# savage-hacker14/audio-to-sheet-music

Hardware: AMD Instinct MI355X
Metric: 6s-segments/sec (each separated into 4 stems; encode once, decode 4x) (higher is better)
Workload: dtype bf16; 1 GPU; BASELINE configs[2]: B=64 x 6 s segments x 4 prompts per GPU; global_batch=64, seq_len=264600, prompts=4, parallelism=segment-sharded dp1, launch=hipGraph replay of one athd_forward_prompts per step (1 graph(s) per rank), pipelines=1, decode_items=256

## Files before the change

### audio-to-sheet-music_amd/csrc/forward.h

```cpp
#pragma once
#include <hip/hip_runtime.h>

#include <algorithm>
#include <cstdio>
#include <cstdlib>
#include <string>
#include <vector>

#include "../../include/athd.h"
#include "attn.h"
#include "ctx.h"
#include "gemm.h"
#include "kernels.h"
#include "prof.h"

namespace athd_fwd {

struct Dims {
    int64_t B = 0, T = 0;
    int P = 1, Tspec = 0;
    int F[5] = {2048, 512, 128, 32, 8};
    int64_t L[5] = {0, 0, 0, 0, 0};
    int64_t Nf = 0, Nt = 0, Nmax = 0;
    int64_t Bc = 0, chunks = 0;
// ... 19 lines not shown
    float *avec, *tc0, *tc2;
    float *Yb, *x_cond, *xt_cond;
    void* Hm;
    float* Ybt;
    void* Hmt;
    float *G, *D, *FO;
    float* FO2 = nullptr;
    float* ola_part;
    LrStep* lrsteps;
    float* gram;
    double* gramq;
    void *S, *Z, *Zs;
    float* skw[2] = {nullptr, nullptr};
};

inline void* eoff(void* p, int64_t n, int ea) { return (char*)p + n * ea; }

struct Switches {
    static bool env(const char* name, bool dflt) {
        const char* e = std::getenv(name);
        return dflt ? !(e && *e == '0') : (e && *e && *e != '0');
    }
    bool serial = env("ATHD_SERIAL", false), sk = env("ATHD_SK", true), rowln = env("ATHD_ROWLN", true),
         fdec1_fused = env("ATHD_FDEC1_FUSED", true), fenc_row = env("ATHD_FENC_ROW", true);
};

struct Status {
    int err = 0;
    std::string what;
    void check(int rc, const char* w) { if (rc != 0 && err == 0) { err = rc; what = w; } }
};

enum Branch { MAIN = 0, TIME = 1 };
struct StreamPlan {
    hipStream_t main, time;
    hipEvent_t ev_f, ev_t;
    bool serial;
    Status* st;

    StreamPlan(athd_ctx* c, hipStream_t caller, bool serial_, Status* st_)
        : main(caller), time(serial_ ? caller : c->s_time), ev_f(c->ev_f), ev_t(c->ev_t), serial(serial_), st(st_) {
        if (!c->s_time || !c->ev_f || !c->ev_t) st->check((int)hipErrorInvalidResourceHandle, "second stream");
    }
    void record(hipEvent_t ev, hipStream_t s) { st->check((int)hipEventRecord(ev, s), "event record"); }
    void wait(hipStream_t s, hipEvent_t ev) { st->check((int)hipStreamWaitEvent(s, ev, 0), "event wait"); }
    void fork() { record(ev_f, main); wait(time, ev_f); }
    void join() { record(ev_t, time); wait(main, ev_t); }
// ... 74 lines not shown
```

### audio-to-sheet-music_amd/csrc/forward_xf.cpp

```cpp
#include "forward.h"

namespace athd_fwd {
namespace {

struct Pending { const double* st = nullptr; const float* w = nullptr; const float* b = nullptr; };

struct BranchX {
    float* X;
    int64_t N;
    void *QKV, *O, *F1;
    Pending pend;
    Pending resgn;
};

struct Xf {
    Run& r;
    const Dims& d;
    const Bufs& b;
    const int ab;

    void ln(BranchX& x, const float* w, const float* bb, bool pending, void* out, const float* w2 = nullptr,
            const float* b2 = nullptr, void* out2 = nullptr) {
        LnDesc l;
        l.x = x.X; l.nb = (int)d.B; l.N = x.N; l.C = 512; l.w = w; l.b = bb; l.out = out; l.out_bf16 = ab;
// ... 49 lines not shown
        GemmDesc g2 = lin(L.l2, x.F1, ab, B, N, 2048, x.X, 0);
        g2.res = x.X; g2.res_scale = L.g2; g2.stats = st;
        g2.sk_ws = r.sw.sk ? b.skw[r.sk] : nullptr;
        r.gemm(g2, "linear2");
        x.pend.st = st; x.pend.w = L.now; x.pend.b = L.nob;
    }
    void down(const GemmW& w, BranchX& x, float* enc, uint16_t* enc_b, const char* site) {
        GemmDesc g = lin(w, x.X, 0, d.B, x.N, 512, enc, 0);
        if (r.actbf) { g.a_gn_stats = x.pend.st; g.a_gn_count = x.N * 512; g.a_gn_w = x.pend.w; g.a_gn_b = x.pend.b; }
        r.gemm(g, site);
        if (enc_b) to_bf16_launch(enc, enc_b, d.B * x.N * 384, r.s);
    }
};

}

void transformer(Run& r, const Dims& d, const Bufs& b) {
    athd_ctx* c = r.c;
    KStage xstage("transformer");
    KSection sec_x("transformer");
    const int64_t B = d.B;
    Xf xf{r, d, b, r.actbf ? 1 : 0};
    BranchX f{b.X, d.Nf, b.QKV, b.O, b.F1}, t{b.XT, d.Nt, b.QKVt, b.Ot, b.F1t};
    r.gemm(lin(c->up, b.saved[3], xf.ab, B, d.Nf, 384, b.X, 0), "upsampler");
    r.gemm(lin(c->up_t, b.saved_t[3], xf.ab, B, d.Nt, 384, b.XT, 0), "upsampler_t");
    pos2d_launch(b.pos2d, 8, d.Tspec, 512, r.s);
    pos1d_launch(b.pos1d, (int)d.Nt, 512, r.s);
    LnDesc l;
    l.x = b.X; l.nb = (int)B; l.N = d.Nf; l.C = 512; l.w = c->nin_w; l.b = c->nin_b; l.pos = b.pos2d; l.out = b.X;
    layernorm_launch(l, r.s);
    LnDesc lt;
    lt.x = b.XT; lt.nb = (int)B; lt.N = d.Nt; lt.C = 512; lt.w = c->nint_w; lt.b = c->nint_b; lt.pos = b.pos1d; lt.out = b.XT;
    layernorm_launch(lt, r.s);
    if (!r.ok()) return;
    r.sp.fork();
    for (int idx = 0; idx < 5; ++idx) {
        const TLayerW& Lf = c->L[idx];
        const TLayerW& Lt = c->Lt[idx];
        if (!Lf.cross) {
            xf.ln(f, Lf.n1w, Lf.n1b, true, b.H[0]);
            xf.block(Lf, f, b.H[0], nullptr, d.Nf);
            OnBranch on(r, TIME);
            xf.ln(t, Lt.n1w, Lt.n1b, true, b.H[2]);
            xf.block(Lt, t, b.H[2], nullptr, d.Nt);
        } else {
            r.sp.cross_join();
            xf.ln(f, Lf.n1w, Lf.n1b, true, b.H[0], Lt.n2w, Lt.n2b, b.H[1]);
            {
                OnBranch on(r, TIME);
                xf.ln(t, Lt.n1w, Lt.n1b, true, b.H[2], Lf.n2w, Lf.n2b, b.H[3]);
            }
            r.sp.cross_join();
            xf.block(Lf, f, b.H[0], b.H[3], d.Nt);
            OnBranch on(r, TIME);
            xf.block(Lt, t, b.H[2], b.H[1], d.Nf);
        }
    }
    if (!r.actbf) gn_apply_launch(b.X, (int)B, d.Nf, 512, f.pend.st, f.pend.w, f.pend.b, r.s);
    {
        OnBranch on(r, TIME);
        if (!r.actbf) gn_apply_launch(b.XT, (int)B, d.Nt, 512, t.pend.st, t.pend.w, t.pend.b, r.s);
        xf.down(c->down_t, t, b.xt_enc, b.xt_enc_b, "downsampler_t");
    }
    xf.down(c->down, f, b.x_enc, b.x_enc_b, "downsampler");
    r.sp.join();
}
// ... 3 lines not shown
```

### audio-to-sheet-music_amd/csrc/gemm.h

```cpp
#pragma once
#include <hip/hip_runtime.h>
#include <stdint.h>

namespace athd {

enum Act { ACT_NONE = 0, ACT_GELU = 1, ACT_GLU = 2 };

struct FastDivU {
    uint32_t mul = 0, shift = 0, d = 1;
};
inline FastDivU make_fastdiv(uint32_t d) {
    FastDivU f;
    f.d = d;
    if (d <= 1) return f;
    uint32_t l = 0;
    while ((1ull << l) < d) ++l;
    f.mul = (uint32_t)((((uint64_t)1 << (31 + l)) + d - 1) / d);
    f.shift = l - 1;
    return f;
}
#if defined(__HIPCC__)
__device__ inline uint32_t fdiv(uint32_t n, const FastDivU& f) { return f.d == 1 ? n : __umulhi(n, f.mul) >> f.shift; }
#endif

// ... 32 lines not shown
    int act = ACT_NONE;
    const void* res = nullptr;
    int res_bf16 = 0;
    const float* res_scale = nullptr;
    const double* res_gn_stats = nullptr;
    int64_t res_gn_count = 0;
    const float* res_gn_w = nullptr;
    const float* res_gn_b = nullptr;
    const float* row_add = nullptr;
    double* stats = nullptr;
    const double* gn_stats = nullptr;
    FastDivU fd_w, fd_h, fd_hw;
    int64_t gn_count = 0;
    const float* gn_w = nullptr;
    const float* gn_b = nullptr;
    const float* pbias = nullptr;
    int pfold = 1, res_div = 1;
    int64_t res_bs = 0;
    const float* ln_w = nullptr;
    const float* ln_b = nullptr;
    void* ln_out = nullptr;
    float* sk_ws = nullptr;
    int sk_full = 0, sk_S = 1;
};

constexpr int SK_MAX_PIECES = 320;
constexpr size_t SK_WS_BYTES = (size_t)SK_MAX_PIECES * 256 * 256 * 4;

inline void gemm_work(const GemmDesc& d, int mode, double& flops, double& bytes) {
    const double M = (double)d.nb * d.H_out * d.W;
    flops = 2.0 * M * d.N * d.K;
    const double nout = d.act == ACT_GLU ? d.N / 2 : d.N;
    bytes = (double)d.nb * d.H_in * d.W * d.C_in * (d.a_bf16 ? 2 : 4) + (double)d.N * d.K * (mode == 1 ? 2 : 4);
    if (d.store) bytes += M * nout * (d.c_bf16 ? 2 : 4) * (d.pfold > 1 ? d.pfold : 1);
    if (d.res) bytes += M * nout * (d.res_bf16 ? 2 : 4) / (d.res_div > 1 ? d.res_div : 1);
    if (d.pbias) bytes += (double)d.nb * (d.pfold > 1 ? d.pfold : 1) * d.N * 4;
}

enum GemmRoute {
    ROUTE_REFUSED = 0,
    ROUTE_ROWLN,
    ROUTE_ROWLN_TEXT,
    ROUTE_GEMM3_LN,
    ROUTE_GEMM2_AGN,
    ROUTE_GEMM5,
    ROUTE_GEMM3_V3,
    ROUTE_GEMM3_V7,
    ROUTE_GEMM2,
    ROUTE_V1_BF16,
    ROUTE_V1_F32
};

int gemm_launch(const GemmDesc& d, int mode, hipStream_t s);
int gemm_route(const GemmDesc& d, int mode);
struct SkPlan {
    int full, tail, S;
};
SkPlan gemm5_sk_plan(const GemmDesc& d, int64_t R);
int64_t gemm5_sk_resident(const GemmDesc& d);
bool rowln_supported(const GemmDesc& d);
inline GemmDesc with_fastdiv(const GemmDesc& d) {
    GemmDesc e = d;
    e.fd_w = make_fastdiv((uint32_t)d.W);
    e.fd_h = make_fastdiv((uint32_t)d.H_out);
    e.fd_hw = make_fastdiv((uint32_t)d.H_out * (uint32_t)d.W);
    return e;
}

}
```

### audio-to-sheet-music_amd/csrc/gemm.hip

```cpp
#include <cstdlib>

#include "gemm_launch.h"

namespace athd {

constexpr int BK = 32;

template <int MODE> struct CT;
template <> struct CT<0> { typedef float T; };
template <> struct CT<1> { typedef bf16_t T; };

typedef __attribute__((ext_vector_type(8))) __bf16 bf16v8;

template <typename T> struct Vec8 { T v[8]; };

template <int MODE, int BM, int BN, int WM, int WN, bool VEC8>
__global__ __launch_bounds__(256) void gemm_kernel(const GemmDesc d) {
    using T = typename CT<MODE>::T;
    constexpr int PAD = (MODE == 1) ? 8 : 4;
    constexpr int LD = BK + PAD;
    constexpr int TM = BM / WM / 16;
    constexpr int TN = BN / WN / 16;
    constexpr int AROWS = BM / 64;
    constexpr int BGROUPS = (BN * 4 + 255) / 256;
// ... 215 lines not shown
}

template <int MODE, int BM, int BN, int WM, int WN>
static void launch_cfg(const GemmDesc& d, hipStream_t s) {
    const int64_t M = (int64_t)d.nb * d.H_out * d.W;
    dim3 grid((unsigned)((M + BM - 1) / BM), (unsigned)((d.N + BN - 1) / BN));
    const bool vec8 = (d.C_in % 8 == 0) && (d.a_ld % 8 == 0) && d.a_cs == 1;
    GemmScope ks(s, d, MODE, "gemm_kernel<%d,%d,%d,%d,%d,%s>", MODE, BM, BN, WM, WN, vec8 ? "true" : "false");
    if (vec8) hipLaunchKernelGGL((gemm_kernel<MODE, BM, BN, WM, WN, true>), grid, dim3(256), 0, s, with_fastdiv(d));
    else hipLaunchKernelGGL((gemm_kernel<MODE, BM, BN, WM, WN, false>), grid, dim3(256), 0, s, with_fastdiv(d));
}

template <int MODE>
static void launch_mode(const GemmDesc& d, hipStream_t s) {
    if (d.N <= 16 && d.act != ACT_GLU) launch_cfg<MODE, 256, 16, 4, 1>(d, s);
    else if (d.N <= 32) launch_cfg<MODE, 256, 32, 4, 1>(d, s);
    else if (d.N <= 64) launch_cfg<MODE, 128, 64, 2, 2>(d, s);
    else launch_cfg<MODE, 128, 128, 2, 2>(d, s);
}

int gemm_route(const GemmDesc& d, int mode) {
    if (d.Kp % BK != 0 || d.Kp < d.K || d.C_in <= 0 || d.N <= 0) return ROUTE_REFUSED;
    if (d.act == ACT_GLU && (d.N % 32 != 0)) return ROUTE_REFUSED;
    if (d.ln_out) return mode == 1 && rowln_supported(d) ? ROUTE_ROWLN : ROUTE_REFUSED;
    if (d.ln_w) {
        if (mode != 1) return ROUTE_REFUSED;
        if (rowln_text_enabled() && rowln_text_supported(d)) return ROUTE_ROWLN_TEXT;
        return gemm3_ln_supported(d) ? ROUTE_GEMM3_LN : ROUTE_REFUSED;
    }
    if (d.a_gn_stats) return mode == 1 && gemm2_supported(d) ? ROUTE_GEMM2_AGN : ROUTE_REFUSED;
    if (d.res_gn_stats && !(mode == 1 && gemm5_supported(d) && d.N % 256 == 0 && epi_res_fast_ok(d))) return ROUTE_REFUSED;
    if (mode == 1 && gemm5_supported(d) && d.N % 256 == 0) return ROUTE_GEMM5;
    if (mode == 1 && gemm3_supported(d) && d.N >= 192) return d.K >= 384 ? ROUTE_GEMM3_V7 : ROUTE_GEMM3_V3;
    if (mode == 1 && gemm2_supported(d)) return ROUTE_GEMM2;
    return mode == 1 ? ROUTE_V1_BF16 : ROUTE_V1_F32;
}

int gemm_launch(const GemmDesc& d0, int mode, hipStream_t s) {
    const GemmDesc d = with_fastdiv(d0);
#ifdef ATHD_KBENCH
    if (mode == 1 && gemm_route(d, mode) >= ROUTE_GEMM5) {
        const int rc = gemm6_launch(d, s);
        if (rc != -2) return rc;
    }
#endif
    const GemmRoute route = (GemmRoute)gemm_route(d, mode);
    switch (route) {
        case ROUTE_ROWLN: return rowln_launch(d, s);
        case ROUTE_ROWLN_TEXT: return rowln_text_launch(d, s);
        case ROUTE_GEMM3_LN: return gemm3_ln_launch(d, s);
        case ROUTE_GEMM2_AGN:
        case ROUTE_GEMM2: return gemm2_launch(d, s);
        case ROUTE_GEMM5: return gemm5_launch(d, s);
        case ROUTE_GEMM3_V3:
        case ROUTE_GEMM3_V7: return gemm3_launch(d, s, route);
        case ROUTE_V1_BF16: launch_mode<1>(d, s); return (int)hipGetLastError();
        case ROUTE_V1_F32: launch_mode<0>(d, s); return (int)hipGetLastError();
        default: return -2;
    }
}

}
```

### audio-to-sheet-music_amd/csrc/gemm_launch.h

```cpp
#pragma once
#include "common.h"
#include "prof.h"
#include "gemm.h"
#include "gemm_epi.h"

#include <type_traits>

namespace athd {

bool gemm2_supported(const GemmDesc& d);
int gemm2_launch(const GemmDesc& d, hipStream_t s);
bool gemm3_supported(const GemmDesc& d);
int gemm3_launch(const GemmDesc& d, hipStream_t s, GemmRoute route);
bool gemm3_ln_supported(const GemmDesc& d);
int gemm3_ln_launch(const GemmDesc& d, hipStream_t s);
bool gemm5_supported(const GemmDesc& d);
int gemm5_launch(const GemmDesc& d, hipStream_t s);
int rowln_launch(const GemmDesc& d, hipStream_t s);
bool rowln_text_enabled();
bool rowln_text_supported(const GemmDesc& d);
int rowln_text_launch(const GemmDesc& d, hipStream_t s);
#ifdef ATHD_KBENCH
int gemm3_variant_launch(const GemmDesc& d, hipStream_t s, int variant);
int gemm4_launch(const GemmDesc& d, hipStream_t s);
int gemm5_probe_launch(const GemmDesc& d, hipStream_t s, int probe);
int gemm6_launch(const GemmDesc& d, hipStream_t s);
#endif

template <auto Kernel>
int64_t resident_blocks(int threads) {
    static int per_cu = 0;
    if (per_cu == 0) {
        (void)hipOccupancyMaxActiveBlocksPerMultiprocessor(&per_cu, Kernel, threads, 0);
        if (per_cu <= 0) per_cu = -1;
    }
    return per_cu > 0 ? (int64_t)per_cu * device_cus() : 0;
}

template <typename Fn>
void dispatch_epi(unsigned flags, Fn&& f) {
    switch (flags) {
// ... 20 lines not shown
```

### audio-to-sheet-music_amd/csrc/ktest.cpp

```cpp
#include <hip/hip_runtime.h>
#include <stdint.h>
#include <string.h>

#include "attn.h"
#include "ctx.h"
#include "gemm.h"
#include "kernels.h"

namespace athd {
bool dconv_conv3_supported(int C, int H, int kp, int64_t L);
bool dconv_apply_supported(int C, int H, int kp, int64_t M);
int dec_merge_run();
int dec_merge_maxp();
int dec_last_const(int which);
int fdec1_gram_wb();
int fdec1_gram_blocks();
}

using namespace athd;

extern "C" {

struct KtGemm {
    void* A; int64_t a_bf16, nb, H_in, W, C_in, a_ld, a_cs, a_bs, a_hs, ntaps, in_stride, in_off, dil, H_out;
    void* a_norm; void* a_gn_stats; int64_t a_gn_count; void* a_gn_w; void* a_gn_b;
    void* Wp; int64_t N, K, Kp; void* bias;
    void* C; int64_t c_bf16, H_out_total, o_stride, o_off, ldo, col_off, c_bs, store; void* c4;
    int64_t col_split, hi_row_off, store_mask, k_blk, act;
    void* res; int64_t res_bf16; void* res_scale; void* res_gn_stats; int64_t res_gn_count; void* res_gn_w; void* res_gn_b;
    void* row_add; void* stats; void* gn_stats; int64_t gn_count; void* gn_w; void* gn_b;
    void* pbias; int64_t pfold, res_div, res_bs;
    void* ln_w; void* ln_b; void* ln_out; void* sk_ws;
};

struct KtAttn {
    void* Q; int64_t q_bf16, q_bs, q_ld, q_off;
    void* K; int64_t k_bf16, k_bs, k_ld, k_off;
    void* V; int64_t v_bf16, v_bs, v_ld, v_off;
    void* O; int64_t o_bf16, o_bs, o_ld;
// ... 258 lines not shown
    d.H_skip2 = (int)k->H_skip2; d.C_skip2 = (int)k->C_skip2;
    return d;
}
int kt_fdec_last(const KtDecLast* k, void* stream) { return fdec_last_launch(to_dl(k), (hipStream_t)stream); }
int kt_tdec_last(const KtDecLast* k, void* stream) { return tdec_last_launch(to_dl(k), (hipStream_t)stream); }
int kt_fdec_tail(const KtDecLast* k, void* stream) { return fdec_tail_launch(to_dl(k), (hipStream_t)stream); }
int kt_tdec_tail(const KtDecLast* k, void* stream) { return tdec_tail_launch(to_dl(k), (hipStream_t)stream); }
int kt_tdec_tail_supported(const KtDecLast* k) { return tdec_tail_supported(to_dl(k)); }
int64_t kt_fl_dc() { return dec_last_const(0); }
int64_t kt_ft_dc() { return dec_last_const(1); }
int64_t kt_tl_in() { return dec_last_const(2); }
int64_t kt_tt_rows() { return dec_last_const(3); }
int64_t kt_dm_run() { return dec_merge_run(); }
int64_t kt_merge_maxp() { return dec_merge_maxp(); }
int64_t kt_g_wb() { return fdec1_gram_wb(); }
int64_t kt_fdec1_gram_blocks() { return fdec1_gram_blocks(); }
int64_t kt_dec_last_fold(const float* w, const float* b, const float* P, const float* pb, int64_t br, float* out) {
    const std::vector<float> f = dec_last_fold(std::vector<float>(w, w + 48 * 4 * 8), std::vector<float>(b, b + 4),
                                               std::vector<float>(P, P + 8), std::vector<float>(pb, pb + 2), (int)br);
    if (out) memcpy(out, f.data(), f.size() * sizeof(float));
    return (int64_t)f.size();
}

int kt_gn_apply(float* x, int64_t nb, int64_t N, int64_t C, const double* stats, const float* w, const float* b,
                void* stream) {
    gn_apply_launch(x, (int)nb, N, (int)C, stats, w, b, (hipStream_t)stream);
    return (int)hipGetLastError();
}

}
```

### audio-to-sheet-music_amd/csrc/rowln.hip

```cpp
#include "gemm_launch.h"
#include "gemm_tile.h"

namespace athd {

namespace {

constexpr int RL_N = 512, RL_K = 512;
constexpr int RT_N = 384, RT_K = 384;
constexpr int RL_NS = 3;
template <int KS, int TN, int AQ>
struct RlSched {
    static constexpr int KT = KS / 2;
    static constexpr int step(int ks) { return (ks + 1 < KS ? TN : 0) + ((ks % 2 == 0 && ks / 2 + 2 < KT) ? AQ : 0); }
    static constexpr int through(int ks) {
        int n = TN + 2 * AQ;
        for (int k = 0; k <= ks; ++k) n += step(k);
        return n;
    }
    static constexpr int pos_b(int k) {
        if (k == 0) return TN;
        return through(k - 2) + TN;
    }
    static constexpr int pos_a(int t) {
        if (t < 2) return TN + (t + 1) * AQ;
        return through(2 * (t - 2) - 1) + TN + AQ;
    }
    static constexpr int wait_b(int ks) { return through(ks) - pos_b(ks); }
    static constexpr int wait_a(int ks) { return through(ks) - pos_a(ks / 2 + 1); }
};

}

#ifndef ATHD_RL_RD
#define ATHD_RL_RD 2
#endif
#ifndef ATHD_RL_PROBE
#define ATHD_RL_PROBE 0
#endif

template <int BM, int NW, int N, int K, bool TEXT>
__global__ __launch_bounds__(64 * NW, 2) void rowln_kernel(const GemmDesc d) {
    constexpr int NT = 64 * NW;
    constexpr int RL_N = N, RL_K = K;
    constexpr int RL_KT = K / 64, RL_KS = K / 32;
    constexpr int RL_PAR = 6 * N;
    constexpr int TM = BM / 16, TN = RL_N / NW / 16;
    constexpr int STAGE = BM * 128;
    constexpr int AP = BM / 8;
    constexpr int AQ = (AP + NW - 1) / NW;
    static_assert(AP * 8 == BM && BM % 16 == 0 && TN * 16 * NW == RL_N && K % 64 == 0, "tile shape");
    static_assert(RL_KS == 16 || RL_KS == 12, "K-steps below");
    using S = RlSched<RL_KS, TN, AQ>;
    __shared__ __attribute__((aligned(1024))) char ring[RL_NS * STAGE];
    __shared__ __attribute__((aligned(16))) float par[RL_PAR];
    __shared__ __attribute__((aligned(16))) float red[2][BM][NW];
    __shared__ __attribute__((aligned(1024))) char sink[AQ * NW > AP ? 1024 : 16];

    const int tid = threadIdx.x, lane = tid & 63;
    const int wave = __builtin_amdgcn_readfirstlane(tid >> 6);
    const int l15 = lane & 15, l4 = lane >> 4;
    const uint32_t M = (uint32_t)d.nb * d.H_out;
    const uint32_t rpb = (uint32_t)d.H_out;
    const int ntm = (int)((M + BM - 1) / BM);
    const int tile = xcd_remap((int)blockIdx.x, (int)gridDim.x);
    if (tile >= ntm) return;
    const uint32_t m0 = (uint32_t)tile * BM, Mend = M;
    const int n0 = TN * 16 * wave;

    const uint32_t b0 = m0 / rpb;
    const uint32_t b1 = (b0 + 1) * rpb < M ? b0 + 1 : b0;
    for (int i = tid; i < RL_PAR; i += NT) {
        const int k = i / RL_N, n = i % RL_N;
        if constexpr (TEXT) {
            const float* src = k == 0 ? d.bias : k == 1 ? (d.pbias ? d.pbias + (int64_t)b0 * RL_N : nullptr)
                             : k == 2 ? (d.pbias ? d.pbias + (int64_t)b1 * RL_N : nullptr) : k == 3 ? nullptr
                             : k == 4 ? d.ln_w : d.ln_b;
            par[i] = src ? src[n] : 0.f;
        } else {
            const float* src = k == 0 ? d.bias : k == 1 ? d.res_scale : k == 2 ? d.res_gn_w : k == 3 ? d.res_gn_b
                                                                         : k == 4 ? d.ln_w : d.ln_b;
            par[i] = src ? src[n] : (k == 1 ? 1.f : 0.f);
        }
    }

    const int lrow = lane >> 3, chunk = swz_chunk(lane);
    const char* zero = reinterpret_cast<const char*>(g_zero_page);
    const char* arow[AQ];
#pragma unroll
    for (int q = 0; q < AQ; ++q) {
        const uint32_t m = m0 + 8 * (wave + NW * q) + lrow;
        arow[q] = m < Mend && wave + NW * q < AP ? (const char*)d.A + ((int64_t)m * RL_K + 8 * chunk) * 2 : nullptr;
    }
    auto dma_a = [&](int kt) {
        char* dst = ring + (kt % RL_NS) * STAGE;
#pragma unroll
        for (int q = 0; q < AQ; ++q) {
            const char* src = arow[q] ? arow[q] + kt * 128 : zero;
            char* to = dst + (wave + NW * q) * 1024;
            if (AQ * NW > AP && wave + NW * q >= AP) to = sink;
// ... 47 lines not shown
        if constexpr (s == 1 && kt + 1 < RL_KT) {                                                                  \
            wait_vm<S::wait_a(ks)>();              \
            __builtin_amdgcn_s_barrier();          \
        }                                                                                                          \
    }
    RL_KSTEP(0) RL_KSTEP(1) RL_KSTEP(2) RL_KSTEP(3) RL_KSTEP(4) RL_KSTEP(5) RL_KSTEP(6) RL_KSTEP(7)
    RL_KSTEP(8) RL_KSTEP(9) RL_KSTEP(10) RL_KSTEP(11)
    if constexpr (RL_KS == 16) {
        RL_KSTEP(12) RL_KSTEP(13) RL_KSTEP(14) RL_KSTEP(15)
    }
#undef RL_KSTEP
#undef load_b
    wait_vm<0>();
    if constexpr (ATHD_RL_PROBE == 1) {
        float t = 0.f;
#pragma unroll
        for (int i = 0; i < TM; ++i)
#pragma unroll
            for (int j = 0; j < TN; ++j) t += acc[i][j][0] + acc[i][j][3];
        if (t == 1234.5f) ((float*)d.res)[m0] = t;
        return;
    }

    float gm0 = 0.f, gr0 = 1.f, gm1 = 0.f, gr1 = 1.f;
    const bool rgn = !TEXT && d.res_gn_stats != nullptr;
    if (rgn) {
        const uint32_t blast = (M - 1) / rpb;
        gn_params(d.res_gn_stats, b0, d.res_gn_count, gm0, gr0);
        gn_params(d.res_gn_stats, b0 + 1 <= blast ? b0 + 1 : blast, d.res_gn_count, gm1, gr1);
    }
    float* X = (float*)d.C;
    const float* R = (const float*)d.res;
    const int cl = n0 + 4 * l4;
    int64_t rb[TM];
#pragma unroll
    for (int i = 0; i < TM; ++i) {
        const uint32_t m = m0 + 16 * i + l15;
        const uint32_t mm = m < Mend ? m : Mend - 1;
        if constexpr (TEXT) {
            const uint32_t b = mm / rpb;
            rb[i] = (d.res_div > 1 ? (int64_t)(b / (uint32_t)d.res_div) * d.res_bs : (int64_t)b * rpb * RL_N) +
                    (int64_t)(mm - b * rpb) * RL_N + cl;
        } else {
            rb[i] = (int64_t)mm * RL_N + cl;
        }
    }
    constexpr int PC = TN % 4 == 0 ? 4 : TN % 3 == 0 ? 3 : 1, NPC = TN / PC, NP = TM * NPC, RD = ATHD_RL_RD;
    static_assert(TN % PC == 0, "residual pieces");
    float4 rr[RD + 1][PC];
    auto load_piece = [&](int p, float4 (&dst)[PC]) {
        const int i = p / NPC, j0 = (p % NPC) * PC;
#pragma unroll
        for (int jj = 0; jj < PC; ++jj) dst[jj] = *reinterpret_cast<const float4*>(R + rb[i] + 16 * (j0 + jj));
    };
#pragma unroll
    for (int p = 0; p < RD; ++p) load_piece(p, rr[p]);
    float rs[TM];
#pragma unroll
    for (int i = 0; i < TM; ++i) rs[i] = 0.f;
#pragma unroll
    for (int p = 0; p < NP; ++p) {
        if (p + RD < NP) load_piece(p + RD, rr[(p + RD) % (RD + 1)]);
        const int i = p / NPC, j0 = (p % NPC) * PC;
        const uint32_t m = m0 + 16 * i + l15;
        const bool second = m >= (b0 + 1) * rpb;
        const float gm = second ? gm1 : gm0, gr = second ? gr1 : gr0;
        float sum = 0.f;
#pragma unroll
        for (int jj = 0; jj < PC; ++jj) {
            const int j = j0 + jj;
            const int c = cl + 16 * j;
            const float4 bi = *reinterpret_cast<const float4*>(&par[c]);
            float4 r = rr[p % (RD + 1)][jj];
            if constexpr (TEXT) {
                const float4 pb = *reinterpret_cast<const float4*>(&par[(second ? 2 : 1) * RL_N + c]);
                acc[i][j][0] = r.x + (acc[i][j][0] + bi.x + pb.x);
                acc[i][j][1] = r.y + (acc[i][j][1] + bi.y + pb.y);
                acc[i][j][2] = r.z + (acc[i][j][2] + bi.z + pb.z);
                acc[i][j][3] = r.w + (acc[i][j][3] + bi.w + pb.w);
                sum += (acc[i][j][0] + acc[i][j][1]) + (acc[i][j][2] + acc[i][j][3]);
                continue;
            }
            const float4 sc = *reinterpret_cast<const float4*>(&par[RL_N + c]);
            if (rgn) {
                const float4 gw = *reinterpret_cast<const float4*>(&par[2 * RL_N + c]);
                const float4 gb = *reinterpret_cast<const float4*>(&par[3 * RL_N + c]);
                r.x = (r.x - gm) * gr * gw.x + gb.x;
                r.y = (r.y - gm) * gr * gw.y + gb.y;
                r.z = (r.z - gm) * gr * gw.z + gb.z;
                r.w = (r.w - gm) * gr * gw.w + gb.w;
            }
            acc[i][j][0] = r.x + sc.x * (acc[i][j][0] + bi.x);
            acc[i][j][1] = r.y + sc.y * (acc[i][j][1] + bi.y);
            acc[i][j][2] = r.z + sc.z * (acc[i][j][2] + bi.z);
            acc[i][j][3] = r.w + sc.w * (acc[i][j][3] + bi.w);
            if (m < Mend)
                *reinterpret_cast<float4*>(X + rb[i] + 16 * j) =
                    make_float4(acc[i][j][0], acc[i][j][1], acc[i][j][2], acc[i][j][3]);
            sum += (acc[i][j][0] + acc[i][j][1]) + (acc[i][j][2] + acc[i][j][3]);
        }
        rs[i] += sum;
        __builtin_amdgcn_sched_barrier(0);
    }
#pragma unroll
    for (int i = 0; i < TM; ++i) {
        rs[i] += __shfl_xor(rs[i], 16, 64);
        rs[i] += __shfl_xor(rs[i], 32, 64);
    }
    auto row_total = [&](int buf, int row) {
        float t = 0.f;
#pragma unroll
        for (int w = 0; w < NW; w += 4) {
            const float4 a = *reinterpret_cast<const float4*>(&red[buf][row][w]);
            t += (a.x + a.y) + (a.z + a.w);
        }
        return t;
    };
    if (l4 == 0) {
#pragma unroll
        for (int i = 0; i < TM; ++i) red[0][16 * i + l15][wave] = rs[i];
    }
    __syncthreads();
    float mean[TM];
#pragma unroll
    for (int i = 0; i < TM; ++i) {
        mean[i] = row_total(0, 16 * i + l15) * (1.f / RL_N);
        float q = 0.f;
#pragma unroll
        for (int j = 0; j < TN; ++j)
#pragma unroll
            for (int e = 0; e < 4; ++e) {
                const float dv = acc[i][j][e] - mean[i];
                q += dv * dv;
            }
        q += __shfl_xor(q, 16, 64);
        q += __shfl_xor(q, 32, 64);
        rs[i] = q;
    }
    if (l4 == 0) {
#pragma unroll
        for (int i = 0; i < TM; ++i) red[1][16 * i + l15][wave] = rs[i];
    }
    __syncthreads();
    bf16_t* Hout = (bf16_t*)(TEXT ? d.C : d.ln_out);
#pragma unroll
    for (int i = 0; i < TM; ++i) {
        const float rstd = 1.f / sqrtf(row_total(1, 16 * i + l15) * (1.f / RL_N) + 1e-5f);
        const uint32_t m = m0 + 16 * i + l15;
        if (m >= Mend) continue;
#pragma unroll
        for (int j = 0; j < TN; ++j) {
            const int c = cl + 16 * j;
            const float4 lw = *reinterpret_cast<const float4*>(&par[4 * RL_N + c]);
            const float4 lb = *reinterpret_cast<const float4*>(&par[5 * RL_N + c]);
            const float y0 = (acc[i][j][0] - mean[i]) * rstd * lw.x + lb.x;
            const float y1 = (acc[i][j][1] - mean[i]) * rstd * lw.y + lb.y;
            const float y2 = (acc[i][j][2] - mean[i]) * rstd * lw.z + lb.z;
            const float y3 = (acc[i][j][3] - mean[i]) * rstd * lw.w + lb.w;
            *reinterpret_cast<uint2*>(Hout + (int64_t)m * RL_N + c) = make_uint2(pack2bf(y0, y1), pack2bf(y2, y3));
        }
    }
}

#ifndef ATHD_RL_BM
#define ATHD_RL_BM 144
#endif
#ifndef ATHD_RL_NW
#define ATHD_RL_NW 8
#endif
constexpr int RL_BM = ATHD_RL_BM, RL_NW = ATHD_RL_NW;

bool rowln_supported(const GemmDesc& d) {
    return d.ln_out && d.ln_w && d.ln_b && d.a_bf16 && d.N == RL_N && d.K == RL_K && d.Kp >= RL_K && d.Kp % 8 == 0 &&
           d.C_in == RL_K && d.a_ld == RL_K && d.ntaps == 1 && d.W == 1 && d.H_in == d.H_out && d.res && !d.res_bf16 &&
           !d.c_bf16 && d.ldo == RL_N && d.col_off == 0 && d.act == ACT_NONE && !d.stats && !d.gn_stats && !d.pbias &&
           !d.row_add && !d.col_split && d.o_stride == 1 && d.o_off == 0 && d.H_out_total == d.H_out && d.c_bs < 0 &&
           d.H_out >= RL_BM && d.res_div <= 1 && !d.a_norm && !d.a_gn_stats && d.a_bs < 0 && d.a_hs < 0 &&
           (!d.res_gn_stats || (d.res_gn_w && d.res_gn_b && d.res_gn_count > 0));
}

int rowln_launch(const GemmDesc& d, hipStream_t s) {
    if (!rowln_supported(d)) return -2;
    const int64_t M = (int64_t)d.nb * d.H_out;
    const int ntm = (int)((M + RL_BM - 1) / RL_BM);
    KScope ks(s);
    if (ks.on()) {
        ks.begin("rowln_kernel", 2.0 * M * RL_N * RL_K,
                 (double)M * RL_K * 2 + (double)RL_N * RL_K * 2 + (double)M * RL_N * (4 + 4 + 2));
    }
    hipLaunchKernelGGL((rowln_kernel<RL_BM, RL_NW, RL_N, RL_K, false>), dim3((unsigned)ntm), dim3(64 * RL_NW), 0, s, d);
    return (int)hipGetLastError();
}

bool rowln_text_enabled() {
    const char* e = getenv("ATHD_RLT");
    return !(e && e[0] == '0');
}

bool rowln_text_supported(const GemmDesc& d) {
    return d.ln_w && d.ln_b && !d.ln_out && d.a_bf16 && d.N == RT_N && d.K == RT_K && d.Kp >= RT_K && d.Kp % 8 == 0 &&
           d.C_in == RT_K && d.a_ld == RT_K && d.ntaps == 1 && d.W == 1 && d.H_in == d.H_out && d.res && !d.res_bf16 &&
           d.c_bf16 && d.store && d.ldo == RT_N && d.col_off == 0 && d.act == ACT_NONE && !d.stats && !d.gn_stats &&
           !d.res_scale && !d.res_gn_stats && !d.row_add && !d.col_split && d.o_stride == 1 && d.o_off == 0 &&
           d.H_out_total == d.H_out && d.c_bs < 0 && d.pfold <= 1 && d.H_out >= RL_BM && d.res_div >= 1 &&
           (d.res_div == 1 || d.res_bs >= (int64_t)d.H_out * RT_N) && !d.a_norm && !d.a_gn_stats && d.a_bs < 0 &&
           d.a_hs < 0;
}

int rowln_text_launch(const GemmDesc& d, hipStream_t s) {
    if (!rowln_text_supported(d)) return -2;
    const int64_t M = (int64_t)d.nb * d.H_out;
    const int ntm = (int)((M + RL_BM - 1) / RL_BM);
    GemmScope ks(s, d, 1, "rowln_kernel<text>");
    hipLaunchKernelGGL((rowln_kernel<RL_BM, RL_NW, RT_N, RT_K, true>), dim3((unsigned)ntm), dim3(64 * RL_NW), 0, s, d);
    return (int)hipGetLastError();
}

}
```

Measured before the change: 1903 segments/s.

## Fuse transformer entry upsampler GEMM with input LayerNorm, positional add and first-layer norm

Adds an ENTRY form of the row-LayerNorm GEMM kernel. It computes the upsampler projection, applies the input LayerNorm, adds the 2D/1D positional encoding, stores the fp32 residual stream, and writes the bf16 layer-0 norm1 output in one pass. This replaces a GEMM, a layernorm kernel and the first layer's separate layernorm on both the frequency and time branches. The time-branch entry GEMM now runs on the time stream after the fork instead of serially before it. It also adds an opt-in persistent-grid variant of rowln (off by default) and test hooks, and adds per-tile branching and extra barriers inside the kernel.

```diff
diff --git a/audio-to-sheet-music_amd/csrc/forward.h b/audio-to-sheet-music_amd/csrc/forward.h
--- a/audio-to-sheet-music_amd/csrc/forward.h
+++ b/audio-to-sheet-music_amd/csrc/forward.h
@@ -65,7 +65,8 @@
         return dflt ? !(e && *e == '0') : (e && *e && *e != '0');
     }
     bool serial = env("ATHD_SERIAL", false), sk = env("ATHD_SK", true), rowln = env("ATHD_ROWLN", true),
-         fdec1_fused = env("ATHD_FDEC1_FUSED", true), fenc_row = env("ATHD_FENC_ROW", true);
+         fdec1_fused = env("ATHD_FDEC1_FUSED", true), fenc_row = env("ATHD_FENC_ROW", true),
+         xf_entry = env("ATHD_XF_ENTRY", true);
 };
 
 struct Status {
diff --git a/audio-to-sheet-music_amd/csrc/forward_xf.cpp b/audio-to-sheet-music_amd/csrc/forward_xf.cpp
--- a/audio-to-sheet-music_amd/csrc/forward_xf.cpp
+++ b/audio-to-sheet-music_amd/csrc/forward_xf.cpp
@@ -95,26 +95,45 @@
     const int64_t B = d.B;
     Xf xf{r, d, b, r.actbf ? 1 : 0};
     BranchX f{b.X, d.Nf, b.QKV, b.O, b.F1}, t{b.XT, d.Nt, b.QKVt, b.Ot, b.F1t};
-    r.gemm(lin(c->up, b.saved[3], xf.ab, B, d.Nf, 384, b.X, 0), "upsampler");
-    r.gemm(lin(c->up_t, b.saved_t[3], xf.ab, B, d.Nt, 384, b.XT, 0), "upsampler_t");
     pos2d_launch(b.pos2d, 8, d.Tspec, 512, r.s);
     pos1d_launch(b.pos1d, (int)d.Nt, 512, r.s);
-    LnDesc l;
-    l.x = b.X; l.nb = (int)B; l.N = d.Nf; l.C = 512; l.w = c->nin_w; l.b = c->nin_b; l.pos = b.pos2d; l.out = b.X;
-    layernorm_launch(l, r.s);
-    LnDesc lt;
-    lt.x = b.XT; lt.nb = (int)B; lt.N = d.Nt; lt.C = 512; lt.w = c->nint_w; lt.b = c->nint_b; lt.pos = b.pos1d; lt.out = b.XT;
-    layernorm_launch(lt, r.s);
+    GemmDesc ef = lin(c->up, b.saved[3], xf.ab, B, d.Nf, 384, b.X, 0);
+    GemmDesc et = lin(c->up_t, b.saved_t[3], xf.ab, B, d.Nt, 384, b.XT, 0);
+    const bool self0 = !c->L[0].cross && !c->Lt[0].cross && r.actbf && r.sw.xf_entry;
+    GemmDesc ff = ef, ft = et;
+    ff.ln_w = c->nin_w; ff.ln_b = c->nin_b; ff.row_pos = b.pos2d;
+    ff.ln2_w = c->L[0].n1w; ff.ln2_b = c->L[0].n1b; ff.ln_out = b.H[0];
+    ft.ln_w = c->nint_w; ft.ln_b = c->nint_b; ft.row_pos = b.pos1d;
+    ft.ln2_w = c->Lt[0].n1w; ft.ln2_b = c->Lt[0].n1b; ft.ln_out = b.H[2];
+    const bool fuse_f = self0 && rowln_entry_supported(ff), fuse_t = self0 && rowln_entry_supported(ft);
+    if (!fuse_f) {
+        r.gemm(ef, "upsampler");
+        LnDesc l;
+        l.x = b.X; l.nb = (int)B; l.N = d.Nf; l.C = 512; l.w = c->nin_w; l.b = c->nin_b; l.pos = b.pos2d; l.out = b.X;
+        layernorm_launch(l, r.s);
+    }
+    if (!fuse_t) {
+        r.gemm(et, "upsampler_t");
+        LnDesc lt;
+        lt.x = b.XT; lt.nb = (int)B; lt.N = d.Nt; lt.C = 512; lt.w = c->nint_w; lt.b = c->nint_b; lt.pos = b.pos1d;
+        lt.out = b.XT;
+        layernorm_launch(lt, r.s);
+    }
     if (!r.ok()) return;
     r.sp.fork();
+    if (fuse_f) r.gemm(ff, "entry.ln");
+    if (fuse_t) {
+        OnBranch on(r, TIME);
+        r.gemm(ft, "entry_t.ln");
+    }
     for (int idx = 0; idx < 5; ++idx) {
         const TLayerW& Lf = c->L[idx];
         const TLayerW& Lt = c->Lt[idx];
         if (!Lf.cross) {
-            xf.ln(f, Lf.n1w, Lf.n1b, true, b.H[0]);
+            if (!(idx == 0 && fuse_f)) xf.ln(f, Lf.n1w, Lf.n1b, true, b.H[0]);
             xf.block(Lf, f, b.H[0], nullptr, d.Nf);
             OnBranch on(r, TIME);
-            xf.ln(t, Lt.n1w, Lt.n1b, true, b.H[2]);
+            if (!(idx == 0 && fuse_t)) xf.ln(t, Lt.n1w, Lt.n1b, true, b.H[2]);
             xf.block(Lt, t, b.H[2], nullptr, d.Nt);
         } else {
             r.sp.cross_join();
diff --git a/audio-to-sheet-music_amd/csrc/gemm.h b/audio-to-sheet-music_amd/csrc/gemm.h
--- a/audio-to-sheet-music_amd/csrc/gemm.h
+++ b/audio-to-sheet-music_amd/csrc/gemm.h
@@ -78,6 +78,9 @@
     void* ln_out = nullptr;
     float* sk_ws = nullptr;
     int sk_full = 0, sk_S = 1;
+    const float* ln2_w = nullptr;
+    const float* ln2_b = nullptr;
+    const float* row_pos = nullptr;
 };
 
 constexpr int SK_MAX_PIECES = 320;
@@ -104,7 +107,8 @@
     ROUTE_GEMM3_V7,
     ROUTE_GEMM2,
     ROUTE_V1_BF16,
-    ROUTE_V1_F32
+    ROUTE_V1_F32,
+    ROUTE_ROWLN_ENTRY
 };
 
 int gemm_launch(const GemmDesc& d, int mode, hipStream_t s);
@@ -115,6 +119,7 @@
 SkPlan gemm5_sk_plan(const GemmDesc& d, int64_t R);
 int64_t gemm5_sk_resident(const GemmDesc& d);
 bool rowln_supported(const GemmDesc& d);
+bool rowln_entry_supported(const GemmDesc& d);
 inline GemmDesc with_fastdiv(const GemmDesc& d) {
     GemmDesc e = d;
     e.fd_w = make_fastdiv((uint32_t)d.W);
diff --git a/audio-to-sheet-music_amd/csrc/gemm.hip b/audio-to-sheet-music_amd/csrc/gemm.hip
--- a/audio-to-sheet-music_amd/csrc/gemm.hip
+++ b/audio-to-sheet-music_amd/csrc/gemm.hip
@@ -261,7 +261,11 @@
 int gemm_route(const GemmDesc& d, int mode) {
     if (d.Kp % BK != 0 || d.Kp < d.K || d.C_in <= 0 || d.N <= 0) return ROUTE_REFUSED;
     if (d.act == ACT_GLU && (d.N % 32 != 0)) return ROUTE_REFUSED;
-    if (d.ln_out) return mode == 1 && rowln_supported(d) ? ROUTE_ROWLN : ROUTE_REFUSED;
+    if (d.ln_out) {
+        if (mode != 1) return ROUTE_REFUSED;
+        if (!d.res && d.ln2_w) return rowln_entry_supported(d) ? ROUTE_ROWLN_ENTRY : ROUTE_REFUSED;
+        return rowln_supported(d) ? ROUTE_ROWLN : ROUTE_REFUSED;
+    }
     if (d.ln_w) {
         if (mode != 1) return ROUTE_REFUSED;
         if (rowln_text_enabled() && rowln_text_supported(d)) return ROUTE_ROWLN_TEXT;
@@ -287,6 +291,7 @@
     switch (route) {
         case ROUTE_ROWLN: return rowln_launch(d, s);
         case ROUTE_ROWLN_TEXT: return rowln_text_launch(d, s);
+        case ROUTE_ROWLN_ENTRY: return rowln_entry_launch(d, s);
         case ROUTE_GEMM3_LN: return gemm3_ln_launch(d, s);
         case ROUTE_GEMM2_AGN:
         case ROUTE_GEMM2: return gemm2_launch(d, s);
diff --git a/audio-to-sheet-music_amd/csrc/gemm_launch.h b/audio-to-sheet-music_amd/csrc/gemm_launch.h
--- a/audio-to-sheet-music_amd/csrc/gemm_launch.h
+++ b/audio-to-sheet-music_amd/csrc/gemm_launch.h
@@ -17,6 +17,10 @@
 bool gemm5_supported(const GemmDesc& d);
 int gemm5_launch(const GemmDesc& d, hipStream_t s);
 int rowln_launch(const GemmDesc& d, hipStream_t s);
+int rowln_entry_launch(const GemmDesc& d, hipStream_t s);
+bool rowln_persist_enabled();
+void rowln_test_grid_cap(int cap);
+void rowln_share_host(uint32_t M, uint32_t G, uint32_t p, uint32_t* out);
 bool rowln_text_enabled();
 bool rowln_text_supported(const GemmDesc& d);
 int rowln_text_launch(const GemmDesc& d, hipStream_t s);
diff --git a/audio-to-sheet-music_amd/csrc/ktest.cpp b/audio-to-sheet-music_amd/csrc/ktest.cpp
--- a/audio-to-sheet-music_amd/csrc/ktest.cpp
+++ b/audio-to-sheet-music_amd/csrc/ktest.cpp
@@ -15,6 +15,8 @@
 int dec_last_const(int which);
 int fdec1_gram_wb();
 int fdec1_gram_blocks();
+void rowln_test_grid_cap(int cap);
+void rowln_share_host(uint32_t M, uint32_t G, uint32_t p, uint32_t* out);
 }
 
 using namespace athd;
@@ -319,6 +321,30 @@
     return (int64_t)f.size();
 }
 
+struct KtRowlnEntry {
+    void* A; void* Wp; void* bias; void* ln_w; void* ln_b; void* ln2_w; void* ln2_b; void* row_pos; void* C; void* ln_out;
+    int64_t nb, rows, Kp;
+};
+int64_t kt_sizeof_rowln_entry() { return (int64_t)sizeof(KtRowlnEntry); }
+static GemmDesc to_entry(const KtRowlnEntry* k) {
+    GemmDesc g;
+    g.A = k->A; g.a_bf16 = 1; g.nb = (int)k->nb; g.H_in = g.H_out = g.H_out_total = (int)k->rows; g.C_in = g.a_ld = 384;
+    g.Wp = k->Wp; g.N = 512; g.K = 384; g.Kp = (int)k->Kp; g.bias = (const float*)k->bias;
+    g.C = k->C; g.ldo = 512;
+    g.ln_w = (const float*)k->ln_w; g.ln_b = (const float*)k->ln_b; g.ln2_w = (const float*)k->ln2_w;
+    g.ln2_b = (const float*)k->ln2_b; g.row_pos = (const float*)k->row_pos; g.ln_out = k->ln_out;
+    return g;
+}
+int kt_rowln_entry(const KtRowlnEntry* k, void* stream) { return gemm_launch(to_entry(k), 1, (hipStream_t)stream); }
+int kt_rowln_entry_route(const KtRowlnEntry* k) { return gemm_route(to_entry(k), 1); }
+int kt_route_rowln_entry() { return (int)ROUTE_ROWLN_ENTRY; }
+void kt_rowln_grid_cap(int64_t cap) { rowln_test_grid_cap((int)cap); }
+void kt_rowln_share(int64_t M, int64_t G, int64_t p, int64_t* out) {
+    uint32_t o[3];
+    rowln_share_host((uint32_t)M, (uint32_t)G, (uint32_t)p, o);
+    out[0] = o[0]; out[1] = o[1]; out[2] = o[2];
+}
+
 int kt_gn_apply(float* x, int64_t nb, int64_t N, int64_t C, const double* stats, const float* w, const float* b,
                 void* stream) {
     gn_apply_launch(x, (int)nb, N, (int)C, stats, w, b, (hipStream_t)stream);
diff --git a/audio-to-sheet-music_amd/csrc/rowln.hip b/audio-to-sheet-music_amd/csrc/rowln.hip
--- a/audio-to-sheet-music_amd/csrc/rowln.hip
+++ b/audio-to-sheet-music_amd/csrc/rowln.hip
@@ -38,8 +38,23 @@
 #define ATHD_RL_PROBE 0
 #endif
 
-template <int BM, int NW, int N, int K, bool TEXT>
+enum RlForm { RL_OUT = 0, RL_TEXT = 1, RL_ENTRY = 2 };
+
+struct RlShare {
+    uint32_t h0, h1, first;
+};
+ATHD_HD RlShare rl_share(uint32_t M, uint32_t hb, uint32_t G, uint32_t p) {
+    const uint64_t HT = (M + hb - 1) / hb;
+    RlShare s;
+    s.h0 = (uint32_t)(p * HT / G);
+    s.h1 = (uint32_t)((p + 1) * HT / G);
+    s.first = (p & 1) ? 1 : 2;
+    return s;
+}
+
+template <int BM, int NW, int N, int K, int FORM, bool PERSIST>
 __global__ __launch_bounds__(64 * NW, 2) void rowln_kernel(const GemmDesc d) {
+    constexpr bool TEXT = FORM == RL_TEXT, ENTRY = FORM == RL_ENTRY;
     constexpr int NT = 64 * NW;
     constexpr int RL_N = N, RL_K = K;
     constexpr int RL_KT = K / 64, RL_KS = K / 32;
@@ -56,25 +71,43 @@
     __shared__ __attribute__((aligned(16))) float red[2][BM][NW];
     __shared__ __attribute__((aligned(1024))) char sink[AQ * NW > AP ? 1024 : 16];
 
-    const int tid = threadIdx.x, lane = tid & 63;
+    const int tid = threadIdx.x;
     const int wave = __builtin_amdgcn_readfirstlane(tid >> 6);
-    const int l15 = lane & 15, l4 = lane >> 4;
     const uint32_t M = (uint32_t)d.nb * d.H_out;
     const uint32_t rpb = (uint32_t)d.H_out;
     const int ntm = (int)((M + BM - 1) / BM);
     const int tile = xcd_remap((int)blockIdx.x, (int)gridDim.x);
-    if (tile >= ntm) return;
-    const uint32_t m0 = (uint32_t)tile * BM, Mend = M;
+    if (!PERSIST && tile >= ntm) return;
     const int n0 = TN * 16 * wave;
-
-    const uint32_t b0 = m0 / rpb;
+    static_assert(!(PERSIST && TEXT), "the text form keeps the one-tile grid (its parameters change per tile)");
+    uint32_t wh = 0, whend = 0, wn = 2;
+    if constexpr (PERSIST) {
+        const RlShare sh = rl_share(M, BM / 2, (uint32_t)gridDim.x, (uint32_t)tile);
+        wh = (uint32_t)__builtin_amdgcn_readfirstlane((int)sh.h0);
+        whend = (uint32_t)__builtin_amdgcn_readfirstlane((int)sh.h1);
+        wn = sh.first;
+        if (wh >= whend) return;
+    }
+    const uint32_t wh0 = wh;
+    for (;;) {
+    int lane = tid & 63;
+    if constexpr (PERSIST) asm volatile("" : "+v"(lane));
+    const int l15 = lane & 15, l4 = lane >> 4;
+    const uint32_t m0 = PERSIST ? wh * (BM / 2) : (uint32_t)tile * BM;
+    const uint32_t Mend = PERSIST ? min(M, (min(wh + wn, whend)) * (BM / 2)) : M;
+
+    const uint32_t b0 = ENTRY || PERSIST ? (uint32_t)__builtin_amdgcn_readfirstlane((int)(m0 / rpb)) : m0 / rpb;
     const uint32_t b1 = (b0 + 1) * rpb < M ? b0 + 1 : b0;
-    for (int i = tid; i < RL_PAR; i += NT) {
+    for (int i = tid; i < (PERSIST && wh != wh0 ? 0 : RL_PAR); i += NT) {
         const int k = i / RL_N, n = i % RL_N;
         if constexpr (TEXT) {
             const float* src = k == 0 ? d.bias : k == 1 ? (d.pbias ? d.pbias + (int64_t)b0 * RL_N : nullptr)
                              : k == 2 ? (d.pbias ? d.pbias + (int64_t)b1 * RL_N : nullptr) : k == 3 ? nullptr
                              : k == 4 ? d.ln_w : d.ln_b;
+            par[i] = src ? src[n] : 0.f;
+        } else if constexpr (ENTRY) {
+            const float* src = k == 0 ? d.bias : k == 1 ? d.ln_w : k == 2 ? d.ln_b : k == 3 ? nullptr
+                             : k == 4 ? d.ln2_w : d.ln2_b;
             par[i] = src ? src[n] : 0.f;
         } else {
             const float* src = k == 0 ? d.bias : k == 1 ? d.res_scale : k == 2 ? d.res_gn_w : k == 3 ? d.res_gn_b
@@ -168,6 +201,76 @@
         return;
     }
 
+    auto row_total = [&](int buf, int row) {
+        float t = 0.f;
+#pragma unroll
+        for (int w = 0; w < NW; w += 4) {
+            const float4 a = *reinterpret_cast<const float4*>(&red[buf][row][w]);
+            t += (a.x + a.y) + (a.z + a.w);
+        }
+        return t;
+    };
+    const int cl = n0 + 4 * l4;
+    float rs[TM];
+    if constexpr (ENTRY) {
+#pragma unroll
+        for (int i = 0; i < TM; ++i) {
+            float sum = 0.f;
+#pragma unroll
+            for (int j = 0; j < TN; ++j) {
+                const float4 bi = *reinterpret_cast<const float4*>(&par[cl + 16 * j]);
+                acc[i][j][0] += bi.x;
+                acc[i][j][1] += bi.y;
+                acc[i][j][2] += bi.z;
+                acc[i][j][3] += bi.w;
+                sum += (acc[i][j][0] + acc[i][j][1]) + (acc[i][j][2] + acc[i][j][3]);
+            }
+            sum += __shfl_xor(sum, 16, 64);
+            sum += __shfl_xor(sum, 32, 64);
+            rs[i] = sum;
+            __builtin_amdgcn_sched_barrier(0);
+        }
+        if (l4 == 0) {
+#pragma unroll
+            for (int i = 0; i < TM; ++i) red[0][16 * i + l15][wave] = rs[i];
+        }
+        __syncthreads();
+#pragma unroll
+        for (int i = 0; i < TM; ++i) {
+            const float mean = row_total(0, 16 * i + l15) * (1.f / RL_N);
+            float q = 0.f;
+#pragma unroll
+            for (int j = 0; j < TN; ++j)
+#pragma unroll
+                for (int e = 0; e < 4; ++e) {
+                    const float dv = acc[i][j][e] - mean;
+                    q += dv * dv;
+                }
+            q += __shfl_xor(q, 16, 64);
+            q += __shfl_xor(q, 32, 64);
+            rs[i] = q;
+            __builtin_amdgcn_sched_barrier(0);
+        }
+        if (l4 == 0) {
+#pragma unroll
+            for (int i = 0; i < TM; ++i) red[1][16 * i + l15][wave] = rs[i];
+        }
+        __syncthreads();
+#pragma unroll
+        for (int i = 0; i < TM; ++i) {
+            const float mean = row_total(0, 16 * i + l15) * (1.f / RL_N);
+            const float rstd = 1.f / sqrtf(row_total(1, 16 * i + l15) * (1.f / RL_N) + 1e-5f);
+#pragma unroll
+            for (int j = 0; j < TN; ++j)
+#pragma unroll
+                for (int e = 0; e < 4; ++e) acc[i][j][e] = (acc[i][j][e] - mean) * rstd;
+#pragma unroll
+            for (int j = 0; j < TN; ++j) asm volatile("" : "+v"(acc[i][j]));
+            __builtin_amdgcn_sched_barrier(0);
+        }
+        __syncthreads();
+    }
+
     float gm0 = 0.f, gr0 = 1.f, gm1 = 0.f, gr1 = 1.f;
     const bool rgn = !TEXT && d.res_gn_stats != nullptr;
     if (rgn) {
@@ -176,14 +279,18 @@
         gn_params(d.res_gn_stats, b0 + 1 <= blast ? b0 + 1 : blast, d.res_gn_count, gm1, gr1);
     }
     float* X = (float*)d.C;
-    const float* R = (const float*)d.res;
-    const int cl = n0 + 4 * l4;
+    uint32_t l15e = (uint32_t)l15;
+    if constexpr (ENTRY) asm volatile("" : "+v"(l15e));
+    float* xrow = X + (int64_t)(m0 + l15e) * RL_N + cl;
+    const float* R = ENTRY ? d.row_pos : (const float*)d.res;
     int64_t rb[TM];
 #pragma unroll
     for (int i = 0; i < TM; ++i) {
-        const uint32_t m = m0 + 16 * i + l15;
+        const uint32_t m = m0 + 16 * i + l15e;
         const uint32_t mm = m < Mend ? m : Mend - 1;
-        if constexpr (TEXT) {
+        if constexpr (ENTRY) {
+            rb[i] = (int64_t)(mm - (mm >= (b0 + 1) * rpb ? b0 + 1 : b0) * rpb) * RL_N + cl;
+        } else if constexpr (TEXT) {
             const uint32_t b = mm / rpb;
             rb[i] = (d.res_div > 1 ? (int64_t)(b / (uint32_t)d.res_div) * d.res_bs : (int64_t)b * rpb * RL_N) +
                     (int64_t)(mm - b * rpb) * RL_N + cl;
@@ -191,7 +298,7 @@
             rb[i] = (int64_t)mm * RL_N + cl;
         }
     }
-    constexpr int PC = TN % 4 == 0 ? 4 : TN % 3 == 0 ? 3 : 1, NPC = TN / PC, NP = TM * NPC, RD = ATHD_RL_RD;
+    constexpr int PC = TN % 4 == 0 ? 4 : TN % 3 == 0 ? 3 : 1, NPC = TN / PC, NP = TM * NPC, RD = ENTRY ? 1 : ATHD_RL_RD;
     static_assert(TN % PC == 0, "residual pieces");
     float4 rr[RD + 1][PC];
     auto load_piece = [&](int p, float4 (&dst)[PC]) {
@@ -201,7 +308,6 @@
     };
 #pragma unroll
     for (int p = 0; p < RD; ++p) load_piece(p, rr[p]);
-    float rs[TM];
 #pragma unroll
     for (int i = 0; i < TM; ++i) rs[i] = 0.f;
 #pragma unroll
@@ -224,6 +330,19 @@
                 acc[i][j][1] = r.y + (acc[i][j][1] + bi.y + pb.y);
                 acc[i][j][2] = r.z + (acc[i][j][2] + bi.z + pb.z);
                 acc[i][j][3] = r.w + (acc[i][j][3] + bi.w + pb.w);
+                sum += (acc[i][j][0] + acc[i][j][1]) + (acc[i][j][2] + acc[i][j][3]);
+                continue;
+            }
+            if constexpr (ENTRY) {
+                const float4 lw = *reinterpret_cast<const float4*>(&par[RL_N + c]);
+                const float4 lb = *reinterpret_cast<const float4*>(&par[2 * RL_N + c]);
+                acc[i][j][0] = acc[i][j][0] * lw.x + lb.x + r.x;
+                acc[i][j][1] = acc[i][j][1] * lw.y + lb.y + r.y;
+                acc[i][j][2] = acc[i][j][2] * lw.z + lb.z + r.z;
+                acc[i][j][3] = acc[i][j][3] * lw.w + lb.w + r.w;
+                if (m < Mend)
+                    *reinterpret_cast<float4*>(xrow + 16 * i * RL_N + 16 * j) =
+                        make_float4(acc[i][j][0], acc[i][j][1], acc[i][j][2], acc[i][j][3]);
                 sum += (acc[i][j][0] + acc[i][j][1]) + (acc[i][j][2] + acc[i][j][3]);
                 continue;
             }
@@ -253,15 +372,6 @@
         rs[i] += __shfl_xor(rs[i], 16, 64);
         rs[i] += __shfl_xor(rs[i], 32, 64);
     }
-    auto row_total = [&](int buf, int row) {
-        float t = 0.f;
-#pragma unroll
-        for (int w = 0; w < NW; w += 4) {
-            const float4 a = *reinterpret_cast<const float4*>(&red[buf][row][w]);
-            t += (a.x + a.y) + (a.z + a.w);
-        }
-        return t;
-    };
     if (l4 == 0) {
 #pragma unroll
         for (int i = 0; i < TM; ++i) red[0][16 * i + l15][wave] = rs[i];
@@ -306,6 +416,11 @@
             *reinterpret_cast<uint2*>(Hout + (int64_t)m * RL_N + c) = make_uint2(pack2bf(y0, y1), pack2bf(y2, y3));
         }
     }
+    if constexpr (!PERSIST) break;
+    wh += wn;
+    wn = 2;
+    if (wh >= whend) break;
+    }
 }
 
 #ifndef ATHD_RL_BM
@@ -322,20 +437,63 @@
            !d.c_bf16 && d.ldo == RL_N && d.col_off == 0 && d.act == ACT_NONE && !d.stats && !d.gn_stats && !d.pbias &&
            !d.row_add && !d.col_split && d.o_stride == 1 && d.o_off == 0 && d.H_out_total == d.H_out && d.c_bs < 0 &&
            d.H_out >= RL_BM && d.res_div <= 1 && !d.a_norm && !d.a_gn_stats && d.a_bs < 0 && d.a_hs < 0 &&
-           (!d.res_gn_stats || (d.res_gn_w && d.res_gn_b && d.res_gn_count > 0));
+           (!d.res_gn_stats || (d.res_gn_w && d.res_gn_b && d.res_gn_count > 0)) && !d.ln2_w && !d.ln2_b && !d.row_pos;
+}
+
+constexpr int RE_K = 384;
+bool rowln_entry_supported(const GemmDesc& d) {
+    return d.ln_out && d.ln_w && d.ln_b && d.ln2_w && d.ln2_b && d.row_pos && d.a_bf16 && d.N == RL_N && d.K == RE_K &&
+           d.Kp >= RE_K && d.Kp % 8 == 0 && d.C_in == RE_K && d.a_ld == RE_K && d.ntaps == 1 && d.W == 1 &&
+           d.H_in == d.H_out && !d.res && !d.res_scale && !d.res_gn_stats && !d.c_bf16 && d.store && d.C &&
+           d.ldo == RL_N && d.col_off == 0 && d.act == ACT_NONE && !d.stats && !d.gn_stats && !d.pbias && !d.row_add &&
+           !d.col_split && d.o_stride == 1 && d.o_off == 0 && d.H_out_total == d.H_out && d.c_bs < 0 &&
+           d.H_out >= RL_BM && d.res_div <= 1 && !d.a_norm && !d.a_gn_stats && d.a_bs < 0 && d.a_hs < 0 && !d.c4;
+}
+
+bool rowln_persist_enabled() {
+    const char* e = getenv("ATHD_RL_PERSIST");
+    return e && e[0] && e[0] != '0';
+}
+namespace {
+int g_rl_grid_cap = 0;
+}
+void rowln_test_grid_cap(int cap) { g_rl_grid_cap = cap; }
+void rowln_share_host(uint32_t M, uint32_t G, uint32_t p, uint32_t* out) {
+    const RlShare sh = rl_share(M, RL_BM / 2, G, p);
+    out[0] = sh.h0; out[1] = sh.h1; out[2] = sh.first;
+}
+
+template <int K, int FORM>
+static int rl_launch(const GemmDesc& d, hipStream_t s, double bytes_per_elem) {
+    const int64_t M = (int64_t)d.nb * d.H_out;
+    const int ntm = (int)((M + RL_BM - 1) / RL_BM);
+    int64_t G = 0;
+    if (rowln_persist_enabled()) {
+        G = resident_blocks<rowln_kernel<RL_BM, RL_NW, RL_N, K, FORM, true>>(64 * RL_NW);
+        if (G > ntm) G = ntm;
+        if (g_rl_grid_cap > 0) G = G > g_rl_grid_cap ? g_rl_grid_cap : G;
+        else G -= G % 8;
+    }
+    KScope ks(s);
+    if (ks.on()) {
+        ks.begin(klabel("rowln_kernel<%d,%d,%d,%d,%d,%s>", RL_BM, RL_NW, RL_N, K, FORM, G > 0 ? "true" : "false"),
+                 2.0 * M * RL_N * K, (double)M * K * 2 + (double)RL_N * K * 2 + (double)M * RL_N * bytes_per_elem);
+    }
+    if (G > 0)
+        hipLaunchKernelGGL((rowln_kernel<RL_BM, RL_NW, RL_N, K, FORM, true>), dim3((unsigned)G), dim3(64 * RL_NW), 0, s, d);
+    else
+        hipLaunchKernelGGL((rowln_kernel<RL_BM, RL_NW, RL_N, K, FORM, false>), dim3((unsigned)ntm), dim3(64 * RL_NW), 0, s, d);
+    return (int)hipGetLastError();
+}
+
+int rowln_entry_launch(const GemmDesc& d, hipStream_t s) {
+    if (!rowln_entry_supported(d)) return -2;
+    return rl_launch<RE_K, RL_ENTRY>(d, s, 4 + 2);
 }
 
 int rowln_launch(const GemmDesc& d, hipStream_t s) {
     if (!rowln_supported(d)) return -2;
-    const int64_t M = (int64_t)d.nb * d.H_out;
-    const int ntm = (int)((M + RL_BM - 1) / RL_BM);
-    KScope ks(s);
-    if (ks.on()) {
-        ks.begin("rowln_kernel", 2.0 * M * RL_N * RL_K,
-                 (double)M * RL_K * 2 + (double)RL_N * RL_K * 2 + (double)M * RL_N * (4 + 4 + 2));
-    }
-    hipLaunchKernelGGL((rowln_kernel<RL_BM, RL_NW, RL_N, RL_K, false>), dim3((unsigned)ntm), dim3(64 * RL_NW), 0, s, d);
-    return (int)hipGetLastError();
+    return rl_launch<RL_K, RL_OUT>(d, s, 4 + 4 + 2);
 }
 
 bool rowln_text_enabled() {
@@ -357,8 +515,8 @@
     if (!rowln_text_supported(d)) return -2;
     const int64_t M = (int64_t)d.nb * d.H_out;
     const int ntm = (int)((M + RL_BM - 1) / RL_BM);
-    GemmScope ks(s, d, 1, "rowln_kernel<text>");
-    hipLaunchKernelGGL((rowln_kernel<RL_BM, RL_NW, RT_N, RT_K, true>), dim3((unsigned)ntm), dim3(64 * RL_NW), 0, s, d);
+    GemmScope ks(s, d, 1, "rowln_kernel<%d,%d,%d,%d,%d,false>", RL_BM, RL_NW, RT_N, RT_K, (int)RL_TEXT);
+    hipLaunchKernelGGL((rowln_kernel<RL_BM, RL_NW, RT_N, RT_K, RL_TEXT, false>), dim3((unsigned)ntm), dim3(64 * RL_NW), 0, s, d);
     return (int)hipGetLastError();
 }
 
```

New measurement: 1927 segments/s, median of 6. About the same (+1.3%).
